# janstenner/DistributedConvRL-PDE-Control

Measured on AMD Instinct MI355X. Metric: env-steps/sec (KS CNAB2 env step + conv actor fwd + DDPG fwd/bwd/update), higher is better.
Workload: dtype f32

## Files before the change

### distributedconvrl-pde-control_amd/csrc/fused3_critic.hpp

```cpp
#pragma once
#include "fused3_layers.hpp"

namespace pdec {

template <int MT, int MTA>
struct CriticLds {
  static constexpr int HP = 16 * MT, HPa = 16 * MTA;
  static constexpr int Wreg = 0;
  static constexpr int sc = Wreg + wreg_floats(MT, MTA);
  static constexpr int sc2 = sc + small_floats(HP);
  static constexpr int sa = sc2 + small_floats(HP);
  static constexpr int saW2 = sa + small_floats(HPa);
  static constexpr int red = saW2 + big_floats(HPa);
  static constexpr int redA = red + 8;
  static constexpr int red5 = redA + 8 * HP;
  static constexpr int end = red5 + 64;
  static_assert(HP * LDP128 + 16 * LDP128 <= wreg_floats(MT, MTA), "pass C images do not fit the big LDS region");
};

template <int MT, int MTA>
__global__ __launch_bounds__(FTHREADS) __attribute__((amdgpu_num_vgpr(112))) void ddpg_critic_fused_kernel(FusedArgs g) {
  extern __shared__ __align__(16) float smem[];
  const int tid = threadIdx.x, w = tid >> 6, l = tid & 63, lr = l & 15, q = l >> 4;
  using Lds = CriticLds<MT, MTA>;
  constexpr int STATS = stats_chunk(MT);
  constexpr int HP = 16 * MT, HPa = 16 * MTA, LDW = HP + LDWPAD, LDWa = HPa + LDWPAD, NW = FTHREADS / 64;
  constexpr int NS = small_floats(HP), NSa = small_floats(HPa), NB = big_floats(HP), NBa = big_floats(HPa);
  float* Wreg = smem + Lds::Wreg;
  float* sc = smem + Lds::sc;
  float* sc2 = smem + Lds::sc2;
  float* sa = smem + Lds::sa;
  float* saW2 = smem + Lds::saW2;
  float* red = smem + Lds::red;
  const SmallLds SCt = carve_small(sc, HP), SC = carve_small(sc2, HP), SA = carve_small(sa, HPa);
  const int ns = g.ns, na = g.na, K0 = ns + na;
  const int col = blockIdx.x * FCOLS + w * 16 + lr;
  const bool valid = col < g.Bu;
  const LiveRows LAt = live_rows<MTA>(ns, g.At.H, g.full_rows), LC = live_rows<MT>(K0, g.C.H, g.full_rows);
  set_wave_prio(g.prio);

  STAMP_RT(11);
  STAMP(0);
  dma_even<NS, NW>(sc, g.Ct.w, w, l);
  dma_even<NSa, NW>(sa, g.At.w, w, l);
  dma_even<NBa, NW>(saW2, g.At.w + g.At.oW2, w, l);
  float xn[4], xq[4];
#pragma unroll
  for (int t = 0; t < 4; ++t) {
    const int row = 4 * t + q;
    xn[t] = (valid && row < ns) ? g.sn[(size_t)col * ns + row] : 0.f;
    float v = 0.f;
    if (valid && row < ns) v = g.s[(size_t)col * ns + row];
    else if (valid && row < K0) v = g.a[(size_t)col * na + (row - ns)];
    xq[t] = v;
  }
  float rv = valid ? g.r[col] : 0.f;
  float tv = valid ? g.t[col] : 0.f;
  float rsum = 0.f;
  if (g.quirk && g.rpart) {
    for (int i = tid; i < g.nrpart; i += FTHREADS) rsum += g.rpart[i];
  } else if (g.quirk && !g.rbar_dev) {
    const int n4 = ((reinterpret_cast<uintptr_t>(g.r) & 15) == 0) ? g.Bu / 4 : 0;
    const f32x4* r4 = reinterpret_cast<const f32x4*>(g.r);
    int i = tid;
    for (; i + 7 * FTHREADS < n4; i += 8 * FTHREADS) {
      f32x4 v[8];
#pragma unroll
      for (int u = 0; u < 8; ++u) v[u] = r4[i + u * FTHREADS];
#pragma unroll
      for (int u = 0; u < 8; ++u) rsum += (v[u][0] + v[u][1]) + (v[u][2] + v[u][3]);
    }
    for (; i < n4; i += FTHREADS) { const f32x4 v = r4[i]; rsum += (v[0] + v[1]) + (v[2] + v[3]); }
    for (int k = 4 * n4 + tid; k < g.Bu; k += FTHREADS) rsum += g.r[k];
  }
  float rbar_in = g.rbar_dev ? g.rbar_dev[0] : 0.f;
  asm volatile("" : "+v"(xn[0]), "+v"(xn[1]), "+v"(xn[2]), "+v"(xn[3]), "+v"(xq[0]), "+v"(xq[1]), "+v"(xq[2]), "+v"(xq[3]),
               "+v"(rv), "+v"(tv), "+v"(rsum), "+v"(rbar_in));
  dma_wait();
  dma_even<NB, NW>(Wreg, g.Ct.w + g.Ct.oW2, w, l);
  dma_even<NS, NW>(sc2, g.C.w, w, l);
  constexpr int N_SC = dma_count<NS, NW>();
  float rbar = block_sum_lds(rsum, red, tid) / (float)g.Bu;
  if (g.rbar_dev) rbar = rbar_in;
  STAMP(1);

  float x[4];
#pragma unroll
  for (int t = 0; t < 4; ++t) x[t] = xn[t];
  float tgt;
  {
    f32x4 ha1[MTA], ha2[MTA];
    layer_in<MTA, 4>(ha1, x, SA, lr, q, LAt);
    layer_hh_live<MTA, MTA, true>(ha2, ha1, saW2, LDWa, SA.b2, lr, q, LAt.mo);
    relu_<MTA>(ha2);
    const float an = tanhf(head<MTA>(ha2, SA.w3, SA.b3[0], q));
#pragma unroll
    for (int t = 0; t < 4; ++t)
      if (4 * t + q == ns) x[t] = valid ? an : 0.f;
    f32x4 h1[MT], h2[MT];
    layer_in<MT, 4>(h1, x, SCt, lr, q, LC);
    dma_wait_but<N_SC>();
    lds_barrier();
    layer_hh<MT, MT, true>(h2, h1, Wreg, LDW, SCt.b2, lr, q);
    relu_<MT>(h2);
    const float qt = head<MT>(h2, SCt.w3, SCt.b3[0], q);
    tgt = g.gamma * (1.f - tv) * qt;
  }
  dma_wait();
  lds_barrier();
  STAMP(2);
  dma_even<NB, NW>(Wreg, g.C.w + g.C.oW2, w, l);
  STAMP(3);
#pragma unroll
  for (int t = 0; t < 4; ++t) x[t] = xq[t];
  f32x4 h1[MT], h2[MT];
  layer_in<MT, 4>(h1, x, SC, lr, q, LC);
  dma_wait();
  lds_barrier();
  layer_hh<MT, MT, true>(h2, h1, Wreg, LDW, SC.b2, lr, q);
  relu_<MT>(h2);
  const float qv = head<MT>(h2, SC.w3, SC.b3[0], q);
  const float c = valid ? tgt - qv : 0.f;
  const float dq = valid ? -(2.f / (float)g.Bu) * ((g.quirk ? rbar : rv) + c) : 0.f;
  const bool rep = valid && q == 0;
  float sv[5] = {rep ? c : 0.f, rep ? c * c : 0.f, rep ? rv : 0.f, rep ? rv * rv : 0.f, rep ? (rv + c) * (rv + c) : 0.f};
  const int nslab = gridDim.x;
  float* Lm = Wreg;
  float* Rm = Wreg + HP * LDP;
  const int cw = (w & 3) * 16 + lr;

  lds_barrier();
  STAMP(4);
  dma_even<NB, NW>(Wreg, g.C.w + g.C.oW2T, w, l);
  f32x4 dz2[MT];
  head_bwd<MT>(dz2, h2, SC.w3, dq, q);
  float a_keep = 0.f;
  {
    float* redA = smem + Lds::redA;
    float* red5 = smem + Lds::red5;
#pragma unroll
    for (int m = 0; m < MT; ++m)
#pragma unroll
      for (int r = 0; r < 4; ++r) {
        const int row = 16 * m + 4 * q + r;
        h2[m][r] = row_sum16((row == g.C.H ? 1.f : h2[m][r]) * dq);
      }
#pragma unroll
    for (int k = 0; k < 5; ++k)
      for (int off = 32; off > 0; off >>= 1) sv[k] += __shfl_xor(sv[k], off);
    if (lr == 0) {
#pragma unroll
      for (int m = 0; m < MT; ++m)
#pragma unroll
        for (int r = 0; r < 4; ++r) redA[w * HP + 16 * m + 4 * q + r] = h2[m][r];
    }
    if (l == 0)
      for (int k = 0; k < 5; ++k) red5[w * 8 + k] = sv[k];
    lds_barrier();
    if (tid < HP) {
#pragma unroll
      for (int ww = 0; ww < NW; ++ww) a_keep += redA[ww * HP + tid];
    } else if (tid >= FTHREADS - 8) {
      if (tid - (FTHREADS - 8) < 5)
        for (int ww = 0; ww < NW; ++ww) a_keep += red5[ww * 8 + tid - (FTHREADS - 8)];
    }
  }
  STAMP(5);
  dma_wait();
  lds_barrier();
  STAMP(6);
  if (tid < HP)
    g.slab[((size_t)(4 * (tid >> 4)) * nslab + blockIdx.x) * 64 + (tid & 15)] = a_keep;
  else if (tid >= FTHREADS - 8)
    g.slab[((size_t)STATS * nslab + blockIdx.x) * 64 + (tid - (FTHREADS - 8))] = a_keep;
  f32x4 dz1[MT];
  layer_hh<MT, MT, false>(dz1, dz2, Wreg, LDW, nullptr, lr, q);
#pragma unroll
  for (int m = 0; m < MT; ++m)
#pragma unroll
    for (int r = 0; r < 4; ++r) dz1[m][r] = h1[m][r] > 0.f ? dz1[m][r] : 0.f;
  STAMP(7);
  {
    float* Lc = Wreg;
    float* Rc = Wreg + HP * LDP128;
    const int cw128 = w * 16 + lr;
    f32x4 accC[((MT + 7) / 8 + 1) & ~1];
    zero_(accC);
    lds_barrier();
    stage_rows_ld<MT>(Lc, LDP128, dz1, cw128, q, -1);
#pragma unroll
    for (int t = 0; t < 4; ++t) {
      const int row = 4 * t + q;
      Rc[row * LDP128 + cw128] = row == K0 ? 1.f : x[t];
    }
    lds_barrier();
    gemm_pass_paired<((MT + 7) / 8 + 1) & ~1, 8>(accC, Lc, Rc, LDP128, MT, 1, w, lr, q);
    store_pass(accC, g.slab, nslab, MT + MT * MT, MT, 1, w, l);
  }
  STAMP(8);
  {
    f32x4 accB[(MT * MT + 7) / 8];
    zero_(accB);
    lds_barrier();
    if ((w >> 2) == 0) {
      stage_rows<MT>(Lm, dz2, cw, q, -1);
      stage_rows<MT>(Rm, h1, cw, q, g.C.H);
    }
    lds_barrier();
    gemm_pass_paired<(MT * MT + 7) / 8, 4>(accB, Lm, Rm, LDP, MT, MT, w, lr, q);
    lds_barrier();
    if ((w >> 2) == 1) {
      stage_rows<MT>(Lm, dz2, cw, q, -1);
      stage_rows<MT>(Rm, h1, cw, q, g.C.H);
    }
    lds_barrier();
    gemm_pass_paired_store<(MT * MT + 7) / 8, 4>(accB, Lm, Rm, LDP, MT, MT, w, lr, q, g.slab, nslab, MT, l);
  }
  STAMP(9);
  STAMP(10);
  STAMP_RT(12);
}

}
```

### distributedconvrl-pde-control_amd/csrc/fused3_layers.hpp

```cpp
#pragma once
#include "fused3_image.hpp"
#include "mfma_blocks.hpp"

namespace pdec {

#define LDP128 136
__host__ __device__ constexpr int actor_stage_floats(int MTA) { return (32 + 4 * 16 * MTA) * LDP128; }
__host__ __device__ constexpr int wreg_floats(int MT, int MTA) {
  const int HP = 16 * MT;
  int a = big_floats(HP), b = 2 * HP * LDP, c = actor_stage_floats(MTA);
  int m = a > b ? a : b;
  return m > c ? m : c;
}

__host__ __device__ constexpr int slab_tiles(int MT) { return MT + MT * MT + MT; }
__host__ __device__ constexpr int stats_chunk(int MT) { return 4 * slab_tiles(MT); }
static inline size_t slab_floats_total(int MT, int nslab) { return ((size_t)stats_chunk(MT) + 1) * nslab * 64; }

template <int NFL, int NW>
__host__ __device__ constexpr int dma_count() { return (NFL / 256 + NW - 1) / NW; }
template <int NFL, int NW>
__device__ __forceinline__ void dma_even(float* dst_lds, const float* src, int w, int l) {
  static_assert(NFL % 256 == 0 && NFL > 0, "dma_even copies whole 1-KiB pieces");
  constexpr int NCH = NFL / 256;
#pragma unroll
  for (int j = 0; j < dma_count<NFL, NW>(); ++j) {
    int c = w + NW * j;
    c = c < NCH ? c : NCH - 1;
    __builtin_amdgcn_global_load_lds((const __attribute__((address_space(1))) void*)(src + (size_t)c * 256 + l * 4),
                                     (__attribute__((address_space(3))) void*)(dst_lds + (size_t)c * 256), 16, 0, 0);
  }
}
template <int N>
__device__ __forceinline__ void dma_wait_but() { asm volatile("s_waitcnt vmcnt(%0)" ::"n"(N) : "memory"); }
__device__ __forceinline__ void dma_wait() { asm volatile("s_waitcnt vmcnt(0)" ::: "memory"); }

__device__ __forceinline__ void lds_barrier() { asm volatile("s_waitcnt lgkmcnt(0)\n\ts_barrier" ::: "memory"); }
__device__ __forceinline__ float block_sum_lds(float v, float* red, int tid) {
  for (int off = 32; off > 0; off >>= 1) v += __shfl_xor(v, off);
  lds_barrier();
  if ((tid & 63) == 0) red[tid >> 6] = v;
  lds_barrier();
  float r = 0.f;
  for (int i = 0; i < FTHREADS / 64; ++i) r += red[i];
  lds_barrier();
  return r;
}

struct LiveRows {
  int kt, mo;
};
template <int MT>
__device__ __forceinline__ LiveRows live_rows(int K0, int H, int full) {
  LiveRows v;
  v.kt = full ? KXP / 4 : (K0 + 3) >> 2;
  v.mo = full ? MT : (H + 15) >> 4;
  return v;
}

template <int MT, int KT>
__device__ __forceinline__ void layer_in(f32x4 (&h)[MT], const float (&x)[KT], const SmallLds& s, int lr, int q, LiveRows lv) {
  const bool last = MT - 1 < lv.mo;
#pragma unroll
  for (int mo = 0; mo < MT; ++mo) {
    const float* b = s.b1 + 16 * mo + 4 * q;
    h[mo] = f32x4{b[0], b[1], b[2], b[3]};
  }
  auto kstep = [&](int t) {
#pragma unroll
    for (int mo = 0; mo < MT - 1; ++mo) h[mo] = mfma4(s.W1[(16 * mo + lr) * LDW1 + 4 * t + q], x[t], h[mo]);
    if (last) h[MT - 1] = mfma4(s.W1[(16 * (MT - 1) + lr) * LDW1 + 4 * t + q], x[t], h[MT - 1]);
  };
  static_assert(KT == 4, "layer_in: four k-steps (KXP input rows)");
  kstep(0);
  if (lv.kt > 1) {
    kstep(1);
    if (lv.kt > 2) {
      kstep(2);
      if (lv.kt > 3) kstep(3);
    }
  }
  if (!last) h[MT - 1] = f32x4{0.f, 0.f, 0.f, 0.f};
  relu_<MT>(h);
}

template <int MTO, int MTI, bool BIAS, int MO0, int MO1>
__device__ __forceinline__ void layer_hh_part(f32x4 (&out)[MTO], const f32x4 (&in)[MTI], const float* W, int ldw,
                                              const float* bias, int lr, int q) {
#pragma unroll
  for (int mo = MO0; mo + 1 < MO1; mo += 2) {
    f32x4 acc0 = {0.f, 0.f, 0.f, 0.f}, acc1 = {0.f, 0.f, 0.f, 0.f};
    if (BIAS) {
      const float* b = bias + 16 * mo + 4 * q;
      acc0 = f32x4{b[0], b[1], b[2], b[3]};
      acc1 = f32x4{b[16], b[17], b[18], b[19]};
    }
    const float* wrow0 = W + (16 * mo + lr) * ldw + 4 * q;
    const float* wrow1 = wrow0 + 16 * ldw;
    f32x4 wa = *reinterpret_cast<const f32x4*>(wrow0);
    f32x4 wb = *reinterpret_cast<const f32x4*>(wrow1);
#pragma unroll
    for (int m = 0; m < MTI; ++m) {
      f32x4 wan = wa, wbn = wb;
      if (m + 1 < MTI) {
        wan = *reinterpret_cast<const f32x4*>(wrow0 + 16 * (m + 1));
        wbn = *reinterpret_cast<const f32x4*>(wrow1 + 16 * (m + 1));
      }
      __builtin_amdgcn_sched_barrier(0);
      mfma4x4_pair(wa, in[m], acc0, wb, in[m], acc1);
      __builtin_amdgcn_sched_barrier(0);
      wa = wan;
      wb = wbn;
    }
    out[mo] = acc0;
    out[mo + 1] = acc1;
  }
#pragma unroll
  for (int mo = MO0 + ((MO1 - MO0) & ~1); mo < MO1; ++mo) {
    f32x4 acc = {0.f, 0.f, 0.f, 0.f};
    if (BIAS) {
      const float* b = bias + 16 * mo + 4 * q;
      acc = f32x4{b[0], b[1], b[2], b[3]};
    }
    const float* wrow = W + (16 * mo + lr) * ldw + 4 * q;
#pragma unroll
    for (int m = 0; m < MTI; ++m) acc = mfma4x4(*reinterpret_cast<const f32x4*>(wrow + 16 * m), in[m], acc);
    out[mo] = acc;
  }
}
template <int MTO, int MTI, bool BIAS>
__device__ __forceinline__ void layer_hh(f32x4 (&out)[MTO], const f32x4 (&in)[MTI], const float* W, int ldw,
                                         const float* bias, int lr, int q) {
  layer_hh_part<MTO, MTI, BIAS, 0, MTO>(out, in, W, ldw, bias, lr, q);
}
template <int MTO, int MTI, bool BIAS>
__device__ __forceinline__ void layer_hh_live(f32x4 (&out)[MTO], const f32x4 (&in)[MTI], const float* W, int ldw,
                                              const float* bias, int lr, int q, int live) {
  static_assert(MTO == MTI, "layer_hh_live: square hidden layers");
  if (MTO == 1 || live >= MTO) {
    layer_hh<MTO, MTI, BIAS>(out, in, W, ldw, bias, lr, q);
    return;
  }
#pragma unroll
  for (int mo = 0; mo < MTO; ++mo) {
    f32x4 acc = {0.f, 0.f, 0.f, 0.f};
    if (mo < live) {
      if (BIAS) {
        const float* b = bias + 16 * mo + 4 * q;
        acc = f32x4{b[0], b[1], b[2], b[3]};
      }
      const float* wrow = W + (16 * mo + lr) * ldw + 4 * q;
#pragma unroll
      for (int m = 0; m < MTI; ++m)
        if (m < live) acc = mfma4x4(*reinterpret_cast<const f32x4*>(wrow + 16 * m), in[m], acc);
    }
    out[mo] = acc;
  }
}

struct FusedArgs {
  FNet A, C, At, Ct;
  const float *s, *a, *r, *t, *sn;
  int Bu, ns, na;
  float gamma;
  int quirk;
  float* slab;
  const float* rpart;
  int nrpart;
  const float* rbar_dev;
  int prio;
  int full_rows;
  unsigned long long* stamps;
};

#define STAMP_AS(k, counter)                                                                  \
  do {                                                                                        \
    if (g.stamps && threadIdx.x == 0) g.stamps[(size_t)blockIdx.x * 16 + (k)] = counter();    \
  } while (0)
#define STAMP(k) STAMP_AS(k, __builtin_amdgcn_s_memtime)
#define STAMP_RT(k) STAMP_AS(k, __builtin_amdgcn_s_memrealtime)

}
```

### distributedconvrl-pde-control_amd/csrc/mlp_mfma.hip

```cpp
#include "common.hpp"
#include "mlp.hpp"
#define KXP 16
#include "fused3_critic.hpp"
#include "fused3_actor.hpp"
#include "fused3_finish.hpp"
#include "fused3_act.hpp"

namespace pdec {

static int mt_of(int H) { return (H + 1 + 15) / 16; }

#define FUSED3_TILES(X) X(9, 2) X(9, 1) X(2, 2) X(2, 1)
#define FUSED3_ACT_TILES(X) X(2) X(1)

template <class F>
static int visit_tiles(int mt, int mta, F&& f) {
#define X(MT_, MTA_) if (mt == MT_ && mta == MTA_) return f(tile_c<MT_>{}, tile_c<MTA_>{});
  FUSED3_TILES(X)
#undef X
  set_error("fused 3-layer pass: no instantiation for %d critic / %d actor tiles", mt, mta);
  return PDEC_E_INVALID;
}
template <class F>
static int visit_act_tiles(int mta, F&& f) {
#define X(MTA_) if (mta == MTA_) return f(tile_c<MTA_>{});
  FUSED3_ACT_TILES(X)
#undef X
  set_error("fused act: no instantiation for %d actor tiles", mta);
  return PDEC_E_INVALID;
}

static int fused_full_rows() {
  const char* e = getenv("PDEC_FUSED_FULL_ROWS");
  return (e && e[0] == '1') ? 1 : 0;
}

static bool fused_disabled() {
  static int v = -1;
  if (v < 0) {
    const char* e = getenv("PDEC_DISABLE_FUSED");
    v = (e && e[0] == '1') ? 1 : 0;
  }
  return v == 1;
}

bool fused_net_supported(const Mlp* M) {
  if (fused_disabled() || M->dtype != PDEC_F32 || M->L != 3) return false;
  if (M->dims[1] != M->dims[2] || M->dims[0] + 1 > KXP || M->dims[3] != 1) return false;
  if (M->acts[0] != PDEC_ACT_RELU || M->acts[1] != PDEC_ACT_RELU) return false;
  const int mt = mt_of(M->dims[1]);
  return mt == 9 || mt == 2 || mt == 1;
}

static bool fused_supported(const Mlp* A, const Mlp* C) {
  if (!fused_net_supported(A) || !fused_net_supported(C)) return false;
  if (C->dims[0] != A->dims[0] + A->dims[3]) return false;
  if (A->acts[2] != PDEC_ACT_TANH || C->acts[2] != PDEC_ACT_IDENTITY) return false;
  const int mt = mt_of(C->dims[1]), mta = mt_of(A->dims[1]);
  bool ok = false;
#define X(MT_, MTA_) ok = ok || (mt == MT_ && mta == MTA_);
  FUSED3_TILES(X)
#undef X
  return ok;
}

static int ensure_prepped(Mlp* M) {
  const FNet f = make_fnet_layout(M->dims[0], M->dims[1]);
  const size_t bytes = (size_t)f.total * 4;
  if (M->fw.bytes < bytes) {
    PDEC_HIP(M->fw.alloc(bytes));
    PDEC_HIP(M->fw_pub[0].alloc(bytes));
    PDEC_HIP(M->fw_pub[1].alloc(bytes));
    M->fw_dirty = true;
  }
  if (M->fw_dirty) {
    ProfScope ps(M, "fused_prep");
    hipLaunchKernelGGL(prep_fused_kernel, dim3((f.total + 255) / 256), dim3(256), 0, M->stream, M->params.as<float>(),
                       M->fw.as<float>(), f);
    PDEC_HIP(hipGetLastError());
    PDEC_HIP(hipMemcpyAsync(M->fw_pub[0].p, M->fw.p, bytes, hipMemcpyDeviceToDevice, M->stream));
    PDEC_HIP(hipMemcpyAsync(M->fw_pub[1].p, M->fw.p, bytes, hipMemcpyDeviceToDevice, M->stream));
    M->fw_dirty = false;
  }
  return PDEC_OK;
}

static FNet fnet_of(const Mlp* M) {
  FNet f = make_fnet_layout(M->dims[0], M->dims[1]);
  f.w = M->fw.as<float>();
  return f;
}

template <int MT, int MTA>
static size_t lds_bytes(bool actor_pass) {
  return (size_t)(actor_pass ? ActorLds<MT, MTA>::end : CriticLds<MT, MTA>::end) * 4;
}

static int read_stamps(Mlp* C, unsigned long long* dev, int grid, double* out13) {
  PDEC_HIP(hipStreamSynchronize(C->stream));
  std::vector<unsigned long long> h((size_t)grid * 16);
  PDEC_HIP(hipMemcpy(h.data(), dev, h.size() * 8, hipMemcpyDeviceToHost));
  double d[10] = {0}, clk = 0;
  for (int b = 0; b < grid; ++b) {
    for (int k = 0; k < 10; ++k) d[k] += (double)(h[b * 16 + k + 1] - h[b * 16 + k]);
    const double rt = (double)(h[b * 16 + 12] - h[b * 16 + 11]);
    if (rt > 0) clk += (double)(h[b * 16 + 10] - h[b * 16]) / rt * 0.1;
  }
  double tot = 0;
  for (int k = 0; k < 10; ++k) { out13[k] = d[k] / grid; tot += out13[k]; }
  out13[10] = tot;
  out13[11] = clk / grid;
  out13[12] = grid;
  return PDEC_OK;
}
static int dump_stamps(Mlp* C, unsigned long long* dev, int grid) {
  double o[13];
  int rc = read_stamps(C, dev, grid, o);
  if (rc) return rc;
  fprintf(stderr, "[pdec stamps] critic pass, mean shader cycles per phase over %d WGs:", grid);
  static const char* nm[10] = {"load+rbar", "target", "loadQ", "fwdQ", "passA", "loadW2T", "dz1", "passC", "passB", "stats"};
  for (int k = 0; k < 10; ++k) fprintf(stderr, " %s=%.0f", nm[k], o[k]);
  fprintf(stderr, " | total=%.0f cycles, clock=%.3f GHz\n", o[10], o[11]);
  return PDEC_OK;
}

static int split_refused() {
  const char* e = getenv("PDEC_SPLIT");
  if (e && e[0] && e[0] != '0') {
    set_error("PDEC_SPLIT=%s: the experimental bf16-split passes no longer exist (HISTORY.md §3.2a); the passes are exact f32", e);
    return PDEC_E_INVALID;
  }
  return PDEC_OK;
}
template <bool ACTOR, int MT, int MTA>
static int launch_pass(Mlp* C, const FusedArgs& g, int grid) {
  if (int rc = split_refused()) return rc;
  const size_t lds = lds_bytes<MT, MTA>(ACTOR);
  auto kern = ACTOR ? ddpg_actor_fused_kernel<MT, MTA> : ddpg_critic_fused_kernel<MT, MTA>;
  const char* label = ACTOR ? "ddpg_actor_fused" : "ddpg_critic_fused";
  static bool attr_set = false;
  if (!attr_set) {
    PDEC_HIP(hipFuncSetAttribute(reinterpret_cast<const void*>(kern), hipFuncAttributeMaxDynamicSharedMemorySize, (int)lds));
    attr_set = true;
  }
  static const bool env_stamps = getenv("PDEC_STAMPS") != nullptr;
  const bool want_stamps = !ACTOR && (env_stamps || C->stamps_armed);
  FusedArgs ga = g;
  if (want_stamps) {
    if (C->stamps.bytes < (size_t)grid * 16 * 8) PDEC_HIP(C->stamps.alloc((size_t)grid * 16 * 8));
    ga.stamps = C->stamps.as<unsigned long long>();
  }
  if (C->prof && C->prof_reps == 1) {
    PDEC_TIMED_LAUNCH(C, label, kern, dim3(grid), dim3(FTHREADS), lds, ga);
  } else {
    ProfScope ps(C, label, true);
    for (int rep = 0; rep < ps.reps; ++rep)
      hipLaunchKernelGGL(kern, dim3(grid), dim3(FTHREADS), lds, C->stream, ga);
  }
  PDEC_HIP(hipGetLastError());
  if (want_stamps && C->stamps_armed) {
    C->stamps_armed = false;
    return read_stamps(C, ga.stamps, grid, C->stamps_last);
  }
  if (want_stamps) return dump_stamps(C, ga.stamps, grid);
  return PDEC_OK;
}

static int ensure_slab(Mlp* M, size_t floats) {
  if (M->fslab.bytes < floats * 4) PDEC_HIP(M->fslab.alloc(floats * 4));
  return PDEC_OK;
}

static int finish_args(Mlp* M, Mlp* Mt, const float* slabs, int nslab, int MT, double grad_scale, int mode, int Bu, int quirk,
                       void* loss_dev, const AdamPolyak* ap, const void* loss_add, FinishArgs* out) {
  FinishArgs g{};
  g.slabs = slabs; g.nslab = nslab; g.K0 = M->dims[0]; g.H = M->dims[1]; g.MT = MT;
  g.grads = M->grads.as<float>(); g.scale = (float)grad_scale; g.mode = mode; g.Bu = Bu; g.quirk = quirk;
  g.loss_out = (float*)loss_dev;
  g.loss_add = (const float*)loss_add;
  g.apply = ap != nullptr;
  g.prio = env_prio("PDEC_PRIO_MFMA", 2);
  if (ap) {
    int rcb = bp_begin(M, ap->b1, ap->b2, &g.bp);
    if (rcb) return rcb;
    g.p = M->params.as<float>(); g.m = M->m.as<float>(); g.v = M->v.as<float>();
    g.fw = M->fw.as<float>();
    g.fwp = M->fw_pub[M->pub ^ 1].as<float>();
    g.lay = make_fnet_layout(M->dims[0], M->dims[1]);
    g.eta = ap->eta; g.b1 = ap->b1; g.b2 = ap->b2; g.eps = ap->eps;
    if (Mt && (float)ap->rho != 1.0f) {
      g.pt = Mt->params.as<float>(); g.fwt = Mt->fw.as<float>();
      const float r = (float)ap->rho;
      g.rho = r; g.omr = 1.0f - r;
    }
  }
  *out = g;
  return PDEC_OK;
}
static void finish_issued(Mlp* M, const AdamPolyak* ap) {
  if (ap) {
    bp_done(M);
    flip(M->pub);
  }
}

static int launch_finish(Mlp* M, Mlp* Mt, const float* slabs, int nslab, int MT, double grad_scale, int mode,
                         int Bu, int quirk, void* loss_dev, const AdamPolyak* ap, const void* loss_add = nullptr) {
  FinishArgs g;
  if (int rc = finish_args(M, Mt, slabs, nslab, MT, grad_scale, mode, Bu, quirk, loss_dev, ap, loss_add, &g)) return rc;
  const int n = M->nparams;
  {
    const char* label = ap ? (nslab > 0 ? "fused_finish" : "fused_apply") : "fused_reduce";
    const bool use_ref = getenv("PDEC_FINISH_REF") != nullptr;
    hipEvent_t& slot = ap ? M->stop_event : M->reduce_event;
    const hipEvent_t ev = slot;
    if (use_ref) {
      const int nblk = nslab > 0 ? 4 * slab_tiles(MT) : (n + 63) / 64;
      hipLaunchKernelGGL(fused_finish_ref_kernel, dim3(nblk), dim3(1024), 0, M->stream, g);
      if (ev) (void)hipEventRecord(ev, M->stream);
    } else {
      const int nblk = nslab > 0 ? 8 * slab_tiles(MT) : (n + FIN_THREADS - 1) / FIN_THREADS;
      if (M->prof) {
        PDEC_TIMED_LAUNCH(M, label, fused_finish_kernel, dim3(nblk), dim3(FIN_THREADS), 0, g);
        if (ev) (void)hipEventRecord(ev, M->stream);
      } else if (ev) {
        hipExtLaunchKernelGGL(fused_finish_kernel, dim3(nblk), dim3(FIN_THREADS), 0, M->stream, nullptr, ev, 0, g);
      } else {
        hipLaunchKernelGGL(fused_finish_kernel, dim3(nblk), dim3(FIN_THREADS), 0, M->stream, g);
      }
    }
    slot = nullptr;
  }
  PDEC_HIP(hipGetLastError());
  finish_issued(M, ap);
  return PDEC_OK;
}

int fused_flush_pending(Mlp* A) {
  PendingFinish& P = A->pend;
  if (!P.on) return PDEC_OK;
  P.on = false;
  if (P.stop) A->stop_event = P.stop;
  P.stop = nullptr;
  return launch_finish(A, nullptr, P.slabs, P.nslab, P.mta, P.scale, 1, P.Bu, 0, P.loss, &P.ap);
}

static int launch_finish_pair(Mlp* C, Mlp* Ct, const float* slabs, int nslab, int MT, double grad_scale, int Bu, int quirk,
                              void* loss_dev, const AdamPolyak* ap, const void* loss_add, Mlp* A) {
  PendingFinish& P = A->pend;
  if (getenv("PDEC_FINISH_REF") != nullptr || C->prof || A->prof || A->stream != C->stream) {
    if (int rc = fused_flush_pending(A)) return rc;
    return launch_finish(C, Ct, slabs, nslab, MT, grad_scale, 0, Bu, quirk, loss_dev, ap, loss_add);
  }
  FinishArgs gc, ga;
  int rc;
  if ((rc = finish_args(C, Ct, slabs, nslab, MT, grad_scale, 0, Bu, quirk, loss_dev, ap, loss_add, &gc))) return rc;
  if ((rc = finish_args(A, nullptr, P.slabs, P.nslab, P.mta, P.scale, 1, P.Bu, 0, P.loss, &P.ap, nullptr, &ga))) return rc;
  const int nc = 8 * slab_tiles(MT), na = 8 * slab_tiles(P.mta);
  const hipEvent_t ev = C->stop_event, eva = P.stop;
  if (ev)
    hipExtLaunchKernelGGL(fused_finish_pair_kernel, dim3(nc + na), dim3(FIN_THREADS), 0, C->stream, nullptr, ev, 0, gc, ga, nc);
  else
    hipLaunchKernelGGL(fused_finish_pair_kernel, dim3(nc + na), dim3(FIN_THREADS), 0, C->stream, gc, ga, nc);
  C->stop_event = nullptr;
  P.on = false;
  P.stop = nullptr;
  ++A->n_paired;
  PDEC_HIP(hipGetLastError());
  if (eva) PDEC_HIP(hipEventRecord(eva, C->stream));
  finish_issued(C, ap);
  finish_issued(A, &P.ap);
  return PDEC_OK;
}

int fused_unpack_published(Mlp* A, float* flat_out, hipStream_t stream) {
  PDEC_REQUIRE(fused_net_supported(A), "fused_unpack_published: not a fused 3-layer network");
  PDEC_REQUIRE_NO_PENDING(A, "fused_unpack_published");
  int rc = ensure_prepped(A);
  if (rc) return rc;
  FNet f = make_fnet_layout(A->dims[0], A->dims[1]);
  PDEC_REQUIRE(A->nparams == flat_offsets(f.K0, f.H).n, "fused_unpack_published: parameter count");
  hipLaunchKernelGGL(unpack_fused_kernel, dim3((A->nparams + 255) / 256), dim3(256), 0, stream, A->fw_pub[A->pub].as<float>(),
                     flat_out, f);
  PDEC_HIP(hipGetLastError());
  return PDEC_OK;
}

#define FUSED3_ACT_MAX_H 31
static bool fused_act_ok(const Mlp* M, int) {
  return fused_net_supported(M) && M->dims[M->L] == 1 && M->dims[1] <= FUSED3_ACT_MAX_H;
}

static int fused_act_plan(const Mlp* A, int* mta, size_t* lds) {
  *mta = mt_of(A->dims[1]);
  *lds = 0;
#define X(MTA_) if (*mta == MTA_) *lds = (size_t)ActLds<MTA_>::end * 4;
  FUSED3_ACT_TILES(X)
#undef X
  PDEC_REQUIRE(A->acts[2] == PDEC_ACT_TANH || A->acts[2] == PDEC_ACT_IDENTITY, "fused act: unsupported output activation");
  PDEC_REQUIRE(*lds != 0 && *lds <= 64 * 1024, "fused act: hidden width %d too large", A->dims[1]);
  return PDEC_OK;
}

static int fused_policy_act(Mlp* A, const void* state, int cols, double act_noise, double act_limit, int learning, uint64_t seed,
                            uint64_t offset, void* actions_out, const uint64_t* ctr_cur, uint64_t* ctr_next, uint64_t ctr_inc) {
  PDEC_REQUIRE_NO_PENDING(A, "fused act");
  int rc = ensure_prepped(A);
  if (rc) return rc;
  FNet f = fnet_of(A);
  f.w = A->fw_pub[A->pub].as<float>();
  int mta = 0;
  size_t lds = 0;
  if ((rc = fused_act_plan(A, &mta, &lds))) return rc;
  const int tanh_out = A->acts[2] == PDEC_ACT_TANH;
  const int prio = env_prio("PDEC_PRIO_ACT", 3);
  const int full_rows = fused_full_rows();
  const dim3 grid((cols + 63) / 64), block(ACT_THREADS);
  rc = visit_act_tiles(mta, [&](auto MTA) {
#define ACT_ARGS(an) f, (const float*)state, cols, A->dims[0], an, (float)act_limit, learning, tanh_out, seed, offset, \
                     (float*)actions_out, ctr_cur, ctr_next, ctr_inc, prio, full_rows
    auto go = [&](auto kern, auto an) {
      if (A->prof) PDEC_TIMED_LAUNCH(A, "policy_act_fused", kern, grid, block, lds, ACT_ARGS(an));
      else hipLaunchKernelGGL(kern, grid, block, lds, A->stream, ACT_ARGS(an));
    };
    if (learning && A->noise_color) go(policy_act_fused_kernel<decltype(MTA)::value, NoiseColor>, noise_color_of(A, act_noise));
    else if (A->noise_scale) go(policy_act_fused_kernel<decltype(MTA)::value, NoiseScale>, noise_scale_of(A));
    else go(policy_act_fused_kernel<decltype(MTA)::value>, (float)act_noise);
#undef ACT_ARGS
    return (int)PDEC_OK;
  });
  if (rc) return rc;
  PDEC_HIP(hipGetLastError());
  return PDEC_OK;
}

static int fused_act_describe(const Mlp* A, char* name, int name_len, int64_t* lds_out) {
  int mta = 0;
  size_t lds = 0;
  if (int rc = fused_act_plan(A, &mta, &lds)) return rc;
  return visit_act_tiles(mta, [&](auto MTA) {
    snprintf(name, name_len, "policy_act_fused_kernel<%d>", decltype(MTA)::value);
    *lds_out = (int64_t)lds;
    return (int)PDEC_OK;
  });
}

static int fused_adam_polyak(Mlp* M, Mlp* Mt, const AdamPolyak& ap) {
  int rc;
  PDEC_REQUIRE_NO_PENDING(M, "fused apply");
  if ((rc = ensure_prepped(M)) || (Mt && (rc = ensure_prepped(Mt)))) return rc;
  return launch_finish(M, Mt, nullptr, 0, mt_of(M->dims[1]), 1.0, 0, 1, 0, nullptr, &ap);
}

static int fused_critic_grads(Mlp* A, Mlp* C, Mlp* At, Mlp* Ct, const void* s, const void* a, const void* r, const void* t,
                              const void* sn, int Bu, double gamma, int quirk, double grad_scale, void* loss_dev,
                              const AdamPolyak* apply, const void* loss_add) {
  int rc;
  if ((rc = ensure_prepped(C)) || (rc = ensure_prepped(At)) || (rc = ensure_prepped(Ct))) return rc;
  const int mt = mt_of(C->dims[1]), mta = mt_of(A->dims[1]);
  const int grid = (Bu + FCOLS - 1) / FCOLS;
  if ((rc = ensure_slab(C, slab_floats_total(mt, grid)))) return rc;
  FusedArgs g{};
  g.C = fnet_of(C); g.At = fnet_of(At); g.Ct = fnet_of(Ct);
  g.s = (const float*)s; g.a = (const float*)a; g.r = (const float*)r; g.t = (const float*)t; g.sn = (const float*)sn;
  g.Bu = Bu; g.ns = A->dims[0]; g.na = 1; g.gamma = (float)gamma; g.quirk = quirk;
  g.slab = C->fslab.as<float>();
  g.prio = env_prio("PDEC_PRIO_MFMA", 2);
  g.full_rows = fused_full_rows();
  if (quirk && C->rpart_ext) {
    g.rpart = C->rpart_ext; g.nrpart = C->rpart_n;
  } else if (quirk && C->rbar_ext) {
    g.rbar_dev = (const float*)C->rbar_ext;
  } else if (quirk && Bu > 256 * FCOLS) {
    float* rb = nullptr;
    if ((rc = launch_rmean(C, (const float*)r, Bu, &rb))) return rc;
    g.rbar_dev = rb;
  }
  C->rbar_ext = nullptr;
  C->rpart_ext = nullptr;
  rc = visit_tiles(mt, mta, [&](auto MT, auto MTA) {
    return launch_pass<false, decltype(MT)::value, decltype(MTA)::value>(C, g, grid);
  });
  if (rc) return rc;
  if (A->pend.on) {
    if (apply) return launch_finish_pair(C, Ct, C->fslab.as<float>(), grid, mt, grad_scale, Bu, quirk, loss_dev, apply, loss_add, A);
    if ((rc = fused_flush_pending(A))) return rc;
  }
  return launch_finish(C, apply ? Ct : nullptr, C->fslab.as<float>(), grid, mt, grad_scale, 0, Bu, quirk, loss_dev, apply,
                       loss_add);
}

static int fused_describe(const Mlp* A, const Mlp* C, bool actor_pass, char* name, int name_len, int64_t* lds) {
  if (int rc = split_refused()) return rc;
  return visit_tiles(mt_of(C->dims[1]), mt_of(A->dims[1]), [&](auto MT, auto MTA) {
    constexpr int mt_ = decltype(MT)::value, mta_ = decltype(MTA)::value;
    snprintf(name, name_len, "%s<%d,%d>", actor_pass ? "ddpg_actor_fused_kernel" : "ddpg_critic_fused_kernel", mt_, mta_);
    *lds = (int64_t)lds_bytes<mt_, mta_>(actor_pass);
    return (int)PDEC_OK;
  });
}

static int fused_actor_grads(Mlp* A, Mlp* C, Mlp* At, const void* s, int Bu, double grad_scale, void* loss_dev,
                             const AdamPolyak* apply) {
  int rc;
  PDEC_REQUIRE_NO_PENDING(A, "fused actor pass");
  if ((rc = ensure_prepped(C)) || (rc = ensure_prepped(A)) || (apply && At && (rc = ensure_prepped(At)))) return rc;
  const int mt = mt_of(C->dims[1]), mta = mt_of(A->dims[1]);
  const int grid = (Bu + FCOLS - 1) / FCOLS;
  if ((rc = ensure_slab(A, slab_floats_total(mta, grid)))) return rc;
  FusedArgs g{};
  g.C = fnet_of(C); g.A = fnet_of(A);
  g.s = (const float*)s; g.Bu = Bu; g.ns = A->dims[0]; g.na = 1;
  g.slab = A->fslab.as<float>();
  g.prio = env_prio("PDEC_PRIO_MFMA", 2);
  g.full_rows = fused_full_rows();
  rc = visit_tiles(mt, mta, [&](auto MT, auto MTA) {
    return launch_pass<true, decltype(MT)::value, decltype(MTA)::value>(C, g, grid);
  });
  if (rc) return rc;
  if (A->defer_finish && apply && (float)apply->rho == 1.0f) {
    PendingFinish& P = A->pend;
    P.on = true;
    P.slabs = A->fslab.as<float>(); P.nslab = grid; P.mta = mta; P.Bu = Bu; P.scale = grad_scale; P.loss = loss_dev; P.ap = *apply;
    P.stop = A->stop_event;
    A->stop_event = nullptr;
    return PDEC_OK;
  }
  return launch_finish(A, apply ? At : nullptr, A->fslab.as<float>(), grid, mta, grad_scale, 1, Bu, 0, loss_dev, apply);
}

#ifndef __HIP_DEVICE_COMPILE__
const FusedFamily fused3_family = {fused_supported,    fused_net_supported, fused_act_ok,      0,
                                   fused_critic_grads, fused_actor_grads,   fused_adam_polyak, fused_policy_act,
                                   fused_describe,     fused_act_describe};
#endif

}
```

Measured before the change: 5.042 million.

## Reuse resident W2 image for critic backward via transposed MFMA reads

The critic backward pass no longer DMA-loads a separate transposed W2 image into LDS. A new layer_hh_t routine computes dz1 straight from the already-resident forward W2 layout, using a lane-permuted, bank-conflict-checked ds_read_b128 access pattern and 4x4 MFMAs. This removes one global-to-LDS weight transfer, a dma_wait and barriers. The pass-A slab store is deferred to after the next existing barrier. The old path stays behind PDEC_FUSED_W2T_REF. The risk is that the new access pattern issues more scalar-element MFMA instructions and LDS reads in the tail tiles.

```diff
diff --git a/distributedconvrl-pde-control_amd/csrc/fused3_critic.hpp b/distributedconvrl-pde-control_amd/csrc/fused3_critic.hpp
--- a/distributedconvrl-pde-control_amd/csrc/fused3_critic.hpp
+++ b/distributedconvrl-pde-control_amd/csrc/fused3_critic.hpp
@@ -18,7 +18,7 @@
   static_assert(HP * LDP128 + 16 * LDP128 <= wreg_floats(MT, MTA), "pass C images do not fit the big LDS region");
 };
 
-template <int MT, int MTA>
+template <int MT, int MTA, bool REF = false>
 __global__ __launch_bounds__(FTHREADS) __attribute__((amdgpu_num_vgpr(112))) void ddpg_critic_fused_kernel(FusedArgs g) {
   extern __shared__ __align__(16) float smem[];
   const int tid = threadIdx.x, w = tid >> 6, l = tid & 63, lr = l & 15, q = l >> 4;
@@ -129,15 +129,26 @@
   float* Rm = Wreg + HP * LDP;
   const int cw = (w & 3) * 16 + lr;
 
-  lds_barrier();
+  float* redA = smem + Lds::redA;
+  float* red5 = smem + Lds::red5;
+  auto pass_a_store = [&]() {
+    float a_keep = 0.f;
+    if (tid < HP) {
+#pragma unroll
+      for (int ww = 0; ww < NW; ++ww) a_keep += redA[ww * HP + tid];
+      g.slab[((size_t)(4 * (tid >> 4)) * nslab + blockIdx.x) * 64 + (tid & 15)] = a_keep;
+    } else if (tid >= FTHREADS - 8) {
+      if (tid - (FTHREADS - 8) < 5)
+        for (int ww = 0; ww < NW; ++ww) a_keep += red5[ww * 8 + tid - (FTHREADS - 8)];
+      g.slab[((size_t)STATS * nslab + blockIdx.x) * 64 + (tid - (FTHREADS - 8))] = a_keep;
+    }
+  };
+  if constexpr (REF) lds_barrier();
   STAMP(4);
-  dma_even<NB, NW>(Wreg, g.C.w + g.C.oW2T, w, l);
+  if constexpr (REF) dma_even<NB, NW>(Wreg, g.C.w + g.C.oW2T, w, l);
   f32x4 dz2[MT];
   head_bwd<MT>(dz2, h2, SC.w3, dq, q);
-  float a_keep = 0.f;
-  {
-    float* redA = smem + Lds::redA;
-    float* red5 = smem + Lds::red5;
+  {
 #pragma unroll
     for (int m = 0; m < MT; ++m)
 #pragma unroll
@@ -156,25 +167,18 @@
     }
     if (l == 0)
       for (int k = 0; k < 5; ++k) red5[w * 8 + k] = sv[k];
-    lds_barrier();
-    if (tid < HP) {
-#pragma unroll
-      for (int ww = 0; ww < NW; ++ww) a_keep += redA[ww * HP + tid];
-    } else if (tid >= FTHREADS - 8) {
-      if (tid - (FTHREADS - 8) < 5)
-        for (int ww = 0; ww < NW; ++ww) a_keep += red5[ww * 8 + tid - (FTHREADS - 8)];
-    }
   }
   STAMP(5);
-  dma_wait();
-  lds_barrier();
   STAMP(6);
-  if (tid < HP)
-    g.slab[((size_t)(4 * (tid >> 4)) * nslab + blockIdx.x) * 64 + (tid & 15)] = a_keep;
-  else if (tid >= FTHREADS - 8)
-    g.slab[((size_t)STATS * nslab + blockIdx.x) * 64 + (tid - (FTHREADS - 8))] = a_keep;
   f32x4 dz1[MT];
-  layer_hh<MT, MT, false>(dz1, dz2, Wreg, LDW, nullptr, lr, q);
+  if constexpr (REF) {
+    dma_wait();
+    lds_barrier();
+    pass_a_store();
+    layer_hh<MT, MT, false>(dz1, dz2, Wreg, LDW, nullptr, lr, q);
+  } else {
+    layer_hh_t<MT>(dz1, dz2, Wreg, lr, q);
+  }
 #pragma unroll
   for (int m = 0; m < MT; ++m)
 #pragma unroll
@@ -187,6 +191,7 @@
     f32x4 accC[((MT + 7) / 8 + 1) & ~1];
     zero_(accC);
     lds_barrier();
+    if constexpr (!REF) pass_a_store();
     stage_rows_ld<MT>(Lc, LDP128, dz1, cw128, q, -1);
 #pragma unroll
     for (int t = 0; t < 4; ++t) {
diff --git a/distributedconvrl-pde-control_amd/csrc/fused3_layers.hpp b/distributedconvrl-pde-control_amd/csrc/fused3_layers.hpp
--- a/distributedconvrl-pde-control_amd/csrc/fused3_layers.hpp
+++ b/distributedconvrl-pde-control_amd/csrc/fused3_layers.hpp
@@ -153,6 +153,111 @@
 #pragma unroll
       for (int m = 0; m < MTI; ++m)
         if (m < live) acc = mfma4x4(*reinterpret_cast<const f32x4*>(wrow + 16 * m), in[m], acc);
+    }
+    out[mo] = acc;
+  }
+}
+
+__host__ __device__ constexpr int hh_t_offset(int ldw, bool wide, int t, int m, int j, int lr, int q) {
+  return (16 * m + 4 * q + j) * ldw + (wide ? 64 * t + 16 * (lr & 3) + 4 * (lr >> 2) : 16 * t + lr);
+}
+template <int MT>
+constexpr bool hh_t_in_bounds() {
+  constexpr int HP = 16 * MT, LDW = HP + LDWPAD;
+  for (int m = 0; m < MT; ++m)
+    for (int j = 0; j < 4; ++j)
+      for (int l = 0; l < 64; ++l) {
+        for (int g = 0; g < MT / 4; ++g) {
+          const int o = hh_t_offset(LDW, true, g, m, j, l & 15, l >> 4);
+          if (o < 0 || o % 4 != 0 || o + 4 > big_floats(HP)) return false;
+        }
+        for (int mo = MT / 4 * 4; mo < MT; ++mo) {
+          const int o = hh_t_offset(LDW, false, mo, m, j, l & 15, l >> 4);
+          if (o < 0 || o + 1 > big_floats(HP)) return false;
+        }
+      }
+  return true;
+}
+__host__ __device__ constexpr int b128_lane_group(int l) {
+  const int h = l & 31;
+  return 2 * (l >> 5) + ((h < 4 || (h >= 12 && h < 16) || (h >= 20 && h < 28)) ? 0 : 1);
+}
+template <int MT>
+constexpr bool hh_t_conflict_free() {
+  constexpr int LDW = 16 * MT + LDWPAD;
+  for (int g = 0; g < (MT / 4 > 0 ? MT / 4 : 1); ++g)
+    for (int m = 0; m < MT; ++m)
+      for (int j = 0; j < 4; ++j) {
+        unsigned seen[4] = {0, 0, 0, 0};
+        for (int l = 0; l < 64; ++l) {
+          const unsigned slot = 1u << (hh_t_offset(LDW, true, g, m, j, l & 15, l >> 4) / 4 % 16);
+          if (seen[b128_lane_group(l)] & slot) return false;
+          seen[b128_lane_group(l)] |= slot;
+        }
+      }
+  return true;
+}
+template <int MT>
+__device__ __forceinline__ void layer_hh_t(f32x4 (&out)[MT], const f32x4 (&in)[MT], const float* W, int lr, int q) {
+  constexpr int LDW = 16 * MT + LDWPAD, NG = MT / 4, NS = 4 * MT;
+  static_assert(hh_t_in_bounds<MT>(), "layer_hh_t reads beyond the weight image");
+  static_assert(hh_t_conflict_free<MT>(), "layer_hh_t: a ds_read_b128 lane group has a bank conflict");
+#pragma unroll
+  for (int g = 0; g < NG; ++g) {
+    f32x4 acc[4];
+    zero_(acc);
+    f32x4 wa = *reinterpret_cast<const f32x4*>(W + hh_t_offset(LDW, true, g, 0, 0, lr, q));
+#pragma unroll
+    for (int s = 0; s < NS; ++s) {
+      f32x4 wn = wa;
+      if (s + 1 < NS) wn = *reinterpret_cast<const f32x4*>(W + hh_t_offset(LDW, true, g, (s + 1) >> 2, (s + 1) & 3, lr, q));
+      __builtin_amdgcn_sched_barrier(0);
+#pragma unroll
+      for (int i = 0; i < 4; ++i) acc[i] = mfma4(wa[i], in[s >> 2][s & 3], acc[i]);
+      __builtin_amdgcn_sched_barrier(0);
+      wa = wn;
+    }
+#pragma unroll
+    for (int r = 0; r < 4; ++r) out[4 * g + r] = f32x4{acc[0][r], acc[1][r], acc[2][r], acc[3][r]};
+  }
+  auto rd = [&](int mo, int m) {
+    f32x4 a;
+#pragma unroll
+    for (int j = 0; j < 4; ++j) a[j] = W[hh_t_offset(LDW, false, mo, m, j, lr, q)];
+    return a;
+  };
+#pragma unroll
+  for (int mo = 4 * NG; mo + 1 < MT; mo += 2) {
+    f32x4 acc0 = {0.f, 0.f, 0.f, 0.f}, acc1 = {0.f, 0.f, 0.f, 0.f};
+    f32x4 wa = rd(mo, 0), wb = rd(mo + 1, 0);
+#pragma unroll
+    for (int m = 0; m < MT; ++m) {
+      f32x4 wan = wa, wbn = wb;
+      if (m + 1 < MT) {
+        wan = rd(mo, m + 1);
+        wbn = rd(mo + 1, m + 1);
+      }
+      __builtin_amdgcn_sched_barrier(0);
+      mfma4x4_pair(wa, in[m], acc0, wb, in[m], acc1);
+      __builtin_amdgcn_sched_barrier(0);
+      wa = wan;
+      wb = wbn;
+    }
+    out[mo] = acc0;
+    out[mo + 1] = acc1;
+  }
+#pragma unroll
+  for (int mo = 4 * NG + ((MT - 4 * NG) & ~1); mo < MT; ++mo) {
+    f32x4 acc = {0.f, 0.f, 0.f, 0.f};
+    f32x4 wa = rd(mo, 0);
+#pragma unroll
+    for (int m = 0; m < MT; ++m) {
+      f32x4 wan = wa;
+      if (m + 1 < MT) wan = rd(mo, m + 1);
+      __builtin_amdgcn_sched_barrier(0);
+      acc = mfma4x4(wa, in[m], acc);
+      __builtin_amdgcn_sched_barrier(0);
+      wa = wan;
     }
     out[mo] = acc;
   }
diff --git a/distributedconvrl-pde-control_amd/csrc/mlp_mfma.hip b/distributedconvrl-pde-control_amd/csrc/mlp_mfma.hip
--- a/distributedconvrl-pde-control_amd/csrc/mlp_mfma.hip
+++ b/distributedconvrl-pde-control_amd/csrc/mlp_mfma.hip
@@ -33,6 +33,11 @@
 static int fused_full_rows() {
   const char* e = getenv("PDEC_FUSED_FULL_ROWS");
   return (e && e[0] == '1') ? 1 : 0;
+}
+
+static bool fused_w2t_ref() {
+  const char* e = getenv("PDEC_FUSED_W2T_REF");
+  return e && e[0] == '1';
 }
 
 static bool fused_disabled() {
@@ -132,11 +137,12 @@
   }
   return PDEC_OK;
 }
-template <bool ACTOR, int MT, int MTA>
+template <bool ACTOR, int MT, int MTA, bool REF = false>
 static int launch_pass(Mlp* C, const FusedArgs& g, int grid) {
   if (int rc = split_refused()) return rc;
+  if (!ACTOR && !REF && fused_w2t_ref()) return launch_pass<ACTOR, MT, MTA, true>(C, g, grid);
   const size_t lds = lds_bytes<MT, MTA>(ACTOR);
-  auto kern = ACTOR ? ddpg_actor_fused_kernel<MT, MTA> : ddpg_critic_fused_kernel<MT, MTA>;
+  auto kern = ACTOR ? ddpg_actor_fused_kernel<MT, MTA> : ddpg_critic_fused_kernel<MT, MTA, REF>;
   const char* label = ACTOR ? "ddpg_actor_fused" : "ddpg_critic_fused";
   static bool attr_set = false;
   if (!attr_set) {
```

Measured after the change: 5.041 million. No clear change (-0.0%).
